# gmh14/tssplat

Measured on AMD Instinct MI355X. Metric: tetrahedra/sec (energy fwd+bwd), higher is better.
Workload: dtype f32

## Files before the change

include/tssplat_amd.h:

```cpp
#ifndef TSSPLAT_AMD_H
#define TSSPLAT_AMD_H

#include <stdint.h>

#ifdef __cplusplus
extern "C" {
#endif

typedef struct tsamd_handle tsamd_handle;

typedef enum tsamd_status {
    TSAMD_OK = 0,
    TSAMD_ERR_INVALID_ARGUMENT = 1,
    TSAMD_ERR_BAD_MESH = 2,
    TSAMD_ERR_NO_DEVICE = 3,
    TSAMD_ERR_HIP = 4,
    TSAMD_ERR_IO = 5,
    TSAMD_ERR_TILING = 6,
    TSAMD_ERR_HOST_ONLY = 7
} tsamd_status;

typedef struct tsamd_options {
    int32_t struct_size;
    int32_t device;
// ... 49 lines not shown
    const float *rest;
} tsamd_tile_view;

const char *tsamd_last_error(void);
const char *tsamd_version(void);
#define TSAMD_ABI_VERSION 3
int32_t tsamd_abi_version(void);

int tsamd_create(const float *rest_xyz, int64_t n_vertices, const int32_t *tets, int64_t n_tets,
                 const tsamd_options *options, tsamd_handle **out);
int tsamd_create_from_veg(const char *path, const tsamd_options *options, tsamd_handle **out);
int tsamd_create_with_operator(const float *rest_xyz, int64_t n_vertices, const int32_t *tets, int64_t n_tets,
                               const int64_t *op_rowptr, const int32_t *op_col, const double *op_val,
                               const tsamd_options *options, tsamd_handle **out);
void tsamd_destroy(tsamd_handle *h);

int64_t tsamd_num_vertices(const tsamd_handle *h);
int64_t tsamd_num_tets(const tsamd_handle *h);
int tsamd_get_plan_info(const tsamd_handle *h, tsamd_plan_info *out);
int tsamd_get_partition_info(const tsamd_handle *h, tsamd_partition_info *out);
int tsamd_get_tile(const tsamd_handle *h, int64_t tile, tsamd_tile_view *out);
int tsamd_get_finish_lists(const tsamd_handle *h, int64_t *n_finish, const int32_t **vid,
                           const int32_t **off, const int32_t **idx);
int tsamd_get_adjacency(const tsamd_handle *h, const int32_t **nbr);

int tsamd_forward(tsamd_handle *h, const float *x_dev, float c1, float c2, int order,
                  void *stream, float *energy_dev);
int tsamd_backward(tsamd_handle *h, const float *x_dev, const float *grad_out_dev, float c1, float c2,
                   int order, void *stream, float *grad_dev);
int tsamd_forward_backward(tsamd_handle *h, const float *x_dev, const float *grad_out_dev, float c1,
                           float c2, int order, void *stream, float *energy_dev, float *grad_dev);
int tsamd_evaluate_dev_coef(tsamd_handle *h, const float *x_dev, const float *grad_out_dev, const float *coef_dev,
                            int order, void *stream, float *energy_dev, float *grad_dev);
typedef struct tsamd_graph tsamd_graph;
int tsamd_graph_create(tsamd_handle *h, const float *x_dev, const float *grad_out_dev, int order, float *energy_dev,
                       float *grad_dev, tsamd_graph **out);
int tsamd_graph_launch(tsamd_graph *graph, float c1, float c2, void *stream);
int tsamd_graph_launch_to(tsamd_graph *graph, float c1, float c2, void *stream, float *energy_copy_dev, float *grad_dev);
void tsamd_graph_destroy(tsamd_graph *graph);

typedef struct tsamd_train_loop tsamd_train_loop;
int64_t tsamd_train_loop_workspace_bytes(int32_t n_iters);
int tsamd_train_loop_create(tsamd_handle *h, float *param_dev, float *grad_dev, float *g1_dev, float *g2_dev, float *energy_ring_dev,
                            void *workspace_dev, int32_t n_iters, tsamd_train_loop **out);
int tsamd_train_loop_launch(tsamd_train_loop *loop, const float *c1, const float *c2, const int32_t *order, float lr, float beta1, float beta2,
                            int64_t first_step, const float *grad_limit, void *stream);
// ... 99 lines not shown
```

tssplat_amd/_capi.py:

```python
from __future__ import annotations

import ctypes as C
import os

from . import _build

_lib = None


class TsamdError(RuntimeError):

    def __init__(self, code: int, message: str):
        super().__init__(f"tssplat_amd error {code}: {message}")
        self.code = code


class Options(C.Structure):
    _fields_ = [
        ("struct_size", C.c_int32),
        ("device", C.c_int32),
        ("lds_budget_bytes", C.c_int32),
        ("max_threads", C.c_int32),
        ("target_owned", C.c_int32),
        ("lane_search_sweeps", C.c_int32),
# ... 34 lines not shown
        ("planes", C.POINTER(C.c_uint32)), ("row_start", C.POINTER(C.c_uint16)),
        ("gvid", C.POINTER(C.c_int32)), ("vdst", C.POINTER(C.c_int32)), ("slot_tet", C.POINTER(C.c_int32)), ("rest", C.POINTER(C.c_float)),
    ]


ABI_VERSION = 3

SIGNATURES = {
    "tsamd_last_error": (C.c_char_p, []),
    "tsamd_version": (C.c_char_p, []),
    "tsamd_abi_version": (C.c_int32, []),
    "tsamd_create": (C.c_int, [C.c_void_p, C.c_int64, C.c_void_p, C.c_int64, C.POINTER(Options), C.POINTER(C.c_void_p)]),
    "tsamd_create_with_operator": (C.c_int, [C.c_void_p, C.c_int64, C.c_void_p, C.c_int64, C.c_void_p, C.c_void_p, C.c_void_p,
                                             C.POINTER(Options), C.POINTER(C.c_void_p)]),
    "tsamd_create_from_veg": (C.c_int, [C.c_char_p, C.POINTER(Options), C.POINTER(C.c_void_p)]),
    "tsamd_destroy": (None, [C.c_void_p]),
    "tsamd_num_vertices": (C.c_int64, [C.c_void_p]),
    "tsamd_num_tets": (C.c_int64, [C.c_void_p]),
    "tsamd_get_plan_info": (C.c_int, [C.c_void_p, C.POINTER(PlanInfo)]),
    "tsamd_get_partition_info": (C.c_int, [C.c_void_p, C.POINTER(PartitionInfo)]),
    "tsamd_get_tile": (C.c_int, [C.c_void_p, C.c_int64, C.POINTER(TileView)]),
    "tsamd_get_finish_lists": (C.c_int, [C.c_void_p, C.POINTER(C.c_int64), C.POINTER(C.POINTER(C.c_int32)),
                                         C.POINTER(C.POINTER(C.c_int32)), C.POINTER(C.POINTER(C.c_int32))]),
    "tsamd_get_adjacency": (C.c_int, [C.c_void_p, C.POINTER(C.POINTER(C.c_int32))]),
    "tsamd_forward": (C.c_int, [C.c_void_p, C.c_void_p, C.c_float, C.c_float, C.c_int, C.c_void_p, C.c_void_p]),
    "tsamd_backward": (C.c_int, [C.c_void_p, C.c_void_p, C.c_void_p, C.c_float, C.c_float, C.c_int, C.c_void_p,
                                 C.c_void_p]),
    "tsamd_forward_backward": (C.c_int, [C.c_void_p, C.c_void_p, C.c_void_p, C.c_float, C.c_float, C.c_int,
                                         C.c_void_p, C.c_void_p, C.c_void_p]),
    "tsamd_evaluate_dev_coef": (C.c_int, [C.c_void_p, C.c_void_p, C.c_void_p, C.c_void_p, C.c_int, C.c_void_p, C.c_void_p,
                                          C.c_void_p]),
    "tsamd_graph_create": (C.c_int, [C.c_void_p, C.c_void_p, C.c_void_p, C.c_int, C.c_void_p, C.c_void_p, C.POINTER(C.c_void_p)]),
    "tsamd_graph_launch": (C.c_int, [C.c_void_p, C.c_float, C.c_float, C.c_void_p]),
    "tsamd_graph_launch_to": (C.c_int, [C.c_void_p, C.c_float, C.c_float, C.c_void_p, C.c_void_p, C.c_void_p]),
    "tsamd_graph_destroy": (None, [C.c_void_p]),
    "tsamd_read_energy_terms": (C.c_int, [C.c_void_p, C.c_void_p, C.POINTER(C.c_double)]),
    "tsamd_set_timing": (C.c_int, [C.c_void_p, C.c_int]),
    "tsamd_get_timing": (C.c_int, [C.c_void_p, C.POINTER(C.c_double), C.POINTER(C.c_double), C.POINTER(C.c_int64)]),
    "tsamd_scale": (C.c_int, [C.c_void_p, C.c_void_p, C.c_void_p, C.c_int64, C.c_void_p]),
    "tsamd_adam_uniform_step": (C.c_int, [C.c_void_p, C.c_void_p, C.c_void_p, C.c_void_p, C.c_int64, C.c_float, C.c_float,
                                        C.c_float, C.c_int64, C.c_float, C.c_void_p, C.c_void_p]),
    "tsamd_grad_limit_workspace_bytes": (C.c_int64, []),
    "tsamd_grad_limit": (C.c_int, [C.c_void_p, C.c_int64, C.c_float, C.c_float, C.c_void_p, C.c_void_p]),
    "tsamd_train_loop_workspace_bytes": (C.c_int64, [C.c_int32]),
    "tsamd_train_loop_create": (C.c_int, [C.c_void_p, C.c_void_p, C.c_void_p, C.c_void_p, C.c_void_p, C.c_void_p, C.c_void_p, C.c_int32,
                                          C.POINTER(C.c_void_p)]),
# ... 128 lines not shown
```

tssplat_amd/csrc/capi.cpp:

```cpp
#include "../../include/tssplat_amd.h"

#include <hip/hip_runtime_api.h>

#include <algorithm>
#include <cmath>
#include <cstdio>
#include <cstdlib>
#include <cstring>
#include <new>
#include <string>
#include <thread>
#include <vector>

#include "capi_common.h"
#include "kernels.h"
#include "plan.h"

namespace {

thread_local std::string g_err;

int fail(int code, const std::string &msg)
{
    g_err = msg;
// ... 60 lines not shown
        for (hipEvent_t e : h->events) (void)hipEventDestroy(e);
    }
    delete h;
}

int to_device(tsamd_handle *h, int device)
{
    int count = 0;
    if (hipGetDeviceCount(&count) != hipSuccess || count <= 0)
        return fail(TSAMD_ERR_NO_DEVICE, "no HIP device is visible (this library has no CPU fallback)");
    if (device < 0) TSAMD_HIP(hipGetDevice(&device));
    if (device >= count) return fail(TSAMD_ERR_INVALID_ARGUMENT, "device ordinal out of range");
    hipDeviceProp_t prop;
    TSAMD_HIP(hipGetDeviceProperties(&prop, device));
    if (size_t(h->plan.lds_bytes) > prop.sharedMemPerBlock && size_t(h->plan.lds_bytes) > prop.maxSharedMemoryPerMultiProcessor)
        return fail(TSAMD_ERR_NO_DEVICE, std::string("device ") + prop.name + " (" + prop.gcnArchName +
                                             ") offers less LDS per workgroup than the plan needs; built for gfx950");
    DeviceGuard g;
    TSAMD_HIP(g.enter(device));
    h->device = device;
    h->host_only = false;
    const tsamd::Plan &P = h->plan;
    int rc;
    if ((rc = upload(h->d_tiles, P.tiles.data(), P.tiles.size(), h->device_bytes))) return rc;
    if (tsamd::planes_paired(P.spt) && !P.tiles.empty()) {
        tsamd::RawVector<uint32_t> image(P.blob.size());
        const int64_t T = int64_t(P.tiles.size());
        const int nthr = int(std::max<int64_t>(1, std::min<int64_t>({int64_t(std::thread::hardware_concurrency()), 64, T / 64 + 1})));
        std::vector<std::thread> pool;
        for (int w = 0; w < nthr; ++w)
            pool.emplace_back([&, w]() {
                for (int64_t t = T * w / nthr; t < T * (w + 1) / nthr; ++t) {
                    const tsamd::TileDesc &d = P.tiles[size_t(t)];
                    const size_t b0 = size_t(d.blob_off / 4), b1 = t + 1 < T ? size_t(P.tiles[size_t(t) + 1].blob_off / 4) : P.blob.size();
                    const size_t np = size_t(P.n_planes) * size_t(d.s_pad);
                    tsamd::interleave_tile_planes(P.blob.data() + b0, image.data() + b0, P.n_planes, d.s_pad, P.spt);
                    std::memcpy(image.data() + b0 + np, P.blob.data() + b0 + np, (b1 - b0 - np) * 4);
                }
            });
        for (auto &th : pool) th.join();
        const size_t head = size_t(P.tiles[0].blob_off / 4);
        if (head) std::memcpy(image.data(), P.blob.data(), head * 4);
        if ((rc = upload(h->d_blob, reinterpret_cast<const uint8_t *>(image.data()), image.size() * 4, h->device_bytes))) return rc;
    } else if ((rc = upload(h->d_blob, reinterpret_cast<const uint8_t *>(P.blob.data()), P.blob.size() * 4, h->device_bytes))) {
        return rc;
    }
    if ((rc = upload(h->d_gvid, P.gvid.data(), P.gvid.size(), h->device_bytes))) return rc;
// ... 17 lines not shown

int create_common(const float *rest, int64_t n, const int32_t *tets, int64_t m, const tsamd_options *o,
                  tsamd_handle **out, const tsamd::ElementOperatorCSR *op = nullptr)
{
    if (!out) return fail(TSAMD_ERR_INVALID_ARGUMENT, "out is null");
    *out = nullptr;
    tsamd_options opt;
    std::memset(&opt, 0, sizeof(opt));
    opt.device = -1;
    if (o) {
        if (o->struct_size != int32_t(sizeof(tsamd_options)))
            return fail(TSAMD_ERR_INVALID_ARGUMENT, "tsamd_options.struct_size does not match this library");
        if (o->abi_version != TSAMD_ABI_VERSION)
            return fail(TSAMD_ERR_INVALID_ARGUMENT, "tsamd_options.abi_version is " + std::to_string(o->abi_version) + ", this library implements ABI " +
                                                        std::to_string(TSAMD_ABI_VERSION) + " (set it to TSAMD_ABI_VERSION of the header you compile against)");
        opt = *o;
    }
    tsamd::PlanOptions po;
    if (opt.lds_budget_bytes > 0) po.lds_budget = opt.lds_budget_bytes;
    if (opt.max_threads > 0) po.max_threads = opt.max_threads;
    po.target_owned = opt.target_owned;
    po.num_threads = opt.num_threads;
    po.conflict_aware = (opt.debug_flags & 2) ? 0 : 1;
    po.lane_search_sweeps = opt.lane_search_sweeps < 0 ? 0 : (opt.lane_search_sweeps == 0 ? 2 : opt.lane_search_sweeps);
    {
        const int spt = opt.slots_per_thread != 0 ? opt.slots_per_thread : tsamd::kSlotsPerLane;
        if (spt < 2 || spt > 4) return fail(TSAMD_ERR_INVALID_ARGUMENT, "slots_per_thread must be 0, 2, 3 or 4");
        if (!tsamd::lane_layout_supported(spt, opt.max_threads > 0 ? opt.max_threads : tsamd::kTileThreads))
            return fail(TSAMD_ERR_INVALID_ARGUMENT, "max_threads exceeds what the tile kernels are compiled for at " + std::to_string(spt) +
                                                        " slots per thread (2: 768, 3: 1024, 4: 768)");
        if (spt != tsamd::kSlotsPerLane && (op || opt.rebuild_dminv == 1))
            return fail(TSAMD_ERR_INVALID_ARGUMENT, "slots_per_thread 3 and 4 are built for the built-in operator with streamed Dm^-1 only");
        po.slots_per_lane = spt;
    }
    if (opt.rebuild_dminv < 0 || opt.rebuild_dminv > 2) return fail(TSAMD_ERR_INVALID_ARGUMENT, "rebuild_dminv must be 0 (auto), 1 (rebuild) or 2 (stream)");
    po.rebuild_dminv = opt.rebuild_dminv == 1 ? 1 : 0;
    tsamd_handle *h = new (std::nothrow) tsamd_handle();
    if (!h) return fail(TSAMD_ERR_INVALID_ARGUMENT, "out of host memory");
    std::string err;
    int rc = 0;
    try {
        rc = tsamd::build_plan(rest, n, tets, m, po, h->plan, err, op);
    } catch (const std::bad_alloc &) {
        rc = TSAMD_ERR_INVALID_ARGUMENT;
        err = "out of host memory while building the plan";
    }
// ... 50 lines not shown
    if (!x && h->plan.n > 0) return fail(TSAMD_ERR_INVALID_ARGUMENT, "x_dev is null");
    return TSAMD_OK;
}

tsamd::EvalArgs eval_args(tsamd_handle *h, const float *x, const float *grad_out, float c1, float c2, int order, float *energy,
                          float *grad, const float *coef)
{
    tsamd::EvalArgs a;
    a.tiles = h->d_tiles;
    a.blob = h->d_blob;
    a.gvid = h->d_gvid;
    a.vdst = h->d_vdst;
    a.fin_vid = h->d_fin_vid;
    a.fin_off = h->d_fin_off;
    a.n_tiles = int64_t(h->plan.tiles.size());
    a.n_finish = int64_t(h->plan.fin_vid.size());
    a.block_threads = h->plan.block_threads;
    a.lds_bytes = h->plan.lds_bytes;
    a.vert_stride = h->plan.vert_stride;
    a.weighted = h->plan.n_planes == tsamd::kPlanesWeighted || h->plan.n_planes == tsamd::kPlanesWeightedSym;
    a.n_planes = h->plan.n_planes;
    a.rebuild = h->plan.n_planes == tsamd::kPlanesRebuild;
    a.spt = h->plan.spt;
    a.x = x;
    a.grad_out = grad_out;
    a.c1 = c1;
    a.c2 = c2;
    a.coef = coef;
    a.order = order;
    a.grad = grad;
    a.stage = h->d_stage;
    a.partials = h->d_partials;
    a.energy = energy;
    a.terms = h->d_terms;
    return a;
}

int evaluate(tsamd_handle *h, const float *x, const float *grad_out, float c1, float c2, int order, void *stream,
             float *energy, float *grad, const float *coef = nullptr)
{
    int rc = check_eval(h, x);
    if (rc) return rc;
    DeviceGuard g;
    TSAMD_HIP(g.enter(h->device));
    const tsamd::EvalArgs a = eval_args(h, x, grad_out, c1, c2, order, energy, grad, coef);
    if (h->timing) {
// ... 95 lines not shown
    if (!h || !out) return fail(TSAMD_ERR_INVALID_ARGUMENT, "null argument");
    const tsamd::Plan &P = h->plan;
    if (tile < 0 || tile >= int64_t(P.tiles.size())) return fail(TSAMD_ERR_INVALID_ARGUMENT, "tile out of range");
    const tsamd::TileDesc &d = P.tiles[size_t(tile)];
    out->n_slots = d.n_slots;
    out->n_owned = d.n_owned;
    out->s_pad = d.s_pad;
    out->n_verts = d.n_verts;
    out->n_excl = d.n_excl;
    out->stage_off = d.stage_off;
    out->n_rows = d.n_rows;
    out->rec_base = d.rec_base;
    out->planes = P.blob.data() + d.blob_off / 4;
    out->row_start = reinterpret_cast<const uint16_t *>(reinterpret_cast<const uint8_t *>(out->planes) + tsamd::tile_rowtab_offset(P.n_planes, d.s_pad));
    out->gvid = P.gvid.data() + d.vert_off;
    out->vdst = P.vdst.data() + d.vert_off;
    out->slot_tet = P.slot_tet.data() + P.slot_base[size_t(tile)];
    out->rest = P.n_planes == tsamd::kPlanesRebuild
                    ? reinterpret_cast<const float *>(reinterpret_cast<const uint8_t *>(out->planes) + tsamd::tile_rest_offset(P.n_planes, d.s_pad))
                    : nullptr;
    return TSAMD_OK;
}

int tsamd_get_finish_lists(const tsamd_handle *h, int64_t *n_finish, const int32_t **vid, const int32_t **off,
                           const int32_t **idx)
{
    if (!h || !n_finish || !vid || !off || !idx) return fail(TSAMD_ERR_INVALID_ARGUMENT, "null argument");
    *n_finish = int64_t(h->plan.fin_vid.size());
    *vid = h->plan.fin_vid.data();
    *off = h->plan.fin_off.data();
    *idx = h->plan.fin_idx.data();
    return TSAMD_OK;
}

int tsamd_get_adjacency(const tsamd_handle *h, const int32_t **nbr)
{
    if (!h || !nbr) return fail(TSAMD_ERR_INVALID_ARGUMENT, "null argument");
    *nbr = h->plan.nbr.data();
    return TSAMD_OK;
}

int tsamd_forward(tsamd_handle *h, const float *x_dev, float c1, float c2, int order, void *stream,
                  float *energy_dev)
{
    if (!energy_dev) return fail(TSAMD_ERR_INVALID_ARGUMENT, "energy_dev is null");
    return evaluate(h, x_dev, nullptr, c1, c2, order, stream, energy_dev, nullptr);
// ... 221 lines not shown
```

tssplat_amd/csrc/kernels.h:

```cpp
#pragma once

#include <hip/hip_runtime_api.h>

#include <cstdint>

#include "plan.h"

namespace tsamd {

struct EvalArgs {
    const TileDesc *tiles;
    const uint8_t *blob;
    const int32_t *gvid, *vdst;
    const int32_t *fin_vid, *fin_off;
    int64_t n_tiles, n_finish;
    int32_t block_threads, lds_bytes;
    int32_t vert_stride = 0;
    bool rebuild = false;
    bool weighted = false;
    int32_t n_planes = 13;
    int32_t spt = kSlotsPerLane;
    const float *x;
    const float *grad_out;
    float c1, c2;
    const float *coef = nullptr;
    int order;
    float *grad;
    float *stage;
    double *partials;
    float *energy;
    double *terms;
};

hipError_t launch_eval(const EvalArgs &a, hipStream_t stream, hipEvent_t *ev = nullptr);
struct EvalGraph;
hipError_t eval_graph_create(const EvalArgs &a, EvalGraph **out);
hipError_t eval_graph_launch(EvalGraph *g, float c1, float c2, hipStream_t stream, float *energy_copy = nullptr, float *grad = nullptr);
void eval_graph_destroy(EvalGraph *g);
struct TrainLoopGraph;
struct TrainLoopStep {
    float c1, c2;
    int order;
    float bias1, bias2, limit;
};
// ... 12 lines not shown
```

tssplat_amd/csrc/kernels.hip:

```cpp
#include <hip/hip_runtime.h>

#include <vector>

#include "kernels.h"

namespace tsamd {
namespace {

constexpr int kWave = 64;

#define SLOT_FENCE() __builtin_amdgcn_sched_barrier(0)
#define STAGE_PRIORITY(n) __builtin_amdgcn_s_setprio(n)
#define UNDEF(x) asm volatile("" : "=v"(x))
typedef uint32_t v4u __attribute__((ext_vector_type(4)));
typedef uint32_t v2u __attribute__((ext_vector_type(2)));

__device__ __forceinline__ float det3(const float *F)
{
    return -F[2] * F[4] * F[6] + F[1] * F[5] * F[6] + F[2] * F[3] * F[7] - F[0] * F[5] * F[7] - F[1] * F[3] * F[8] +
           F[0] * F[4] * F[8];
}

__device__ __forceinline__ void cof3(const float *F, float *C)
{
// ... 173 lines not shown
    const int32_t *gvid;
    const int32_t *vdst;
    const float *x;
    const float *grad_out;
    float *grad;
    float *stage;
    double *partials;
    float c1, c2;
    float ratio;
    const float *coef;
    int order;
    int n_tiles;
    int tiles_per_xcd;
    int vert_stride;
    int n_planes;
};

constexpr uint32_t kXS = kRowTabBytes;
constexpr uint32_t kZeroEntry = 4u * 66u;

__device__ __forceinline__ uint32_t pos_lo(uint32_t w) { return (w & kVertMask) << 4; }
__device__ __forceinline__ uint32_t pos_hi(uint32_t w) { return ((w >> 16) & kVertMask) << 4; }

template <bool WITH_GRAD, bool WEIGHTED, bool REBUILD, int SPT>
__device__ __forceinline__ void tile_body(const KernelArgs &a, const int tile, int32_t gv0)
{
    extern __shared__ __attribute__((aligned(16))) unsigned char smem[];
    typedef uint32_t VU __attribute__((ext_vector_type(SPT)));
    typedef float VF __attribute__((ext_vector_type(SPT)));
    static_assert(!(REBUILD && WEIGHTED), "rebuild_dminv is built for the built-in operator");
    constexpr int kKeepF = SPT, kKeepH = WEIGHTED ? 0 : SPT;
    const TileDesc td = a.tiles[tile];
    const int tid = threadIdx.x, nthr = blockDim.x;
    typedef const __attribute__((address_space(4))) float *ConstF;
    const float k_c1 = a.coef ? ((ConstF)(uintptr_t)a.coef)[0] : a.c1, k_c2 = a.coef ? ((ConstF)(uintptr_t)a.coef)[1] : a.c2;
    const float grad_out_scale = WITH_GRAD && a.grad_out ? *(ConstF)(uintptr_t)a.grad_out : 1.f;
    const auto g_blob = as_global(a.blob);
    const auto g_gvid = as_global(a.gvid);
    const auto g_vdst = as_global(a.vdst);
    const auto g_x = as_global(a.x);
    const auto g_grad = as_global(a.grad);
    const auto g_stage = as_global(a.stage);
    const auto g_partials = as_global(a.partials);
    const uint32_t VP = uint32_t(td.n_verts + 3) & ~3u;
    const uint32_t RS = kXS + 16u * VP;
    const uint32_t RB = uint32_t(td.rec_base);
    LDS_AS double *red = lds_at<double>(RB - 256u);
    const int nq = td.s_pad / SPT;
    const bool active = tid < nq;
    const GLOBAL_AS uint32_t *pl = reinterpret_cast<const GLOBAL_AS uint32_t *>(g_blob + td.blob_off);
    const int lt = active ? tid : 0;
    typedef VU PlaneU __attribute__((aligned(SPT == 3 ? 4 : 4 * SPT)));
    typedef VF PlaneF __attribute__((aligned(SPT == 3 ? 4 : 4 * SPT)));
    auto plane_u = [&](int q) -> VU { return __builtin_nontemporal_load(reinterpret_cast<const GLOBAL_AS PlaneU *>(pl + q * td.s_pad + SPT * lt)); };
    auto plane_f = [&](int q) -> VF { return __builtin_nontemporal_load(reinterpret_cast<const GLOBAL_AS PlaneF *>(pl + q * td.s_pad + SPT * lt)); };
    constexpr bool kPaired = planes_paired(SPT);
    typedef uint32_t VU2 __attribute__((ext_vector_type(2 * SPT)));
    typedef float VF2 __attribute__((ext_vector_type(2 * SPT)));
    auto pair_u = [&](int q, VU &lo, VU &hi) {
        if (kPaired) {
            const VU2 t = __builtin_nontemporal_load(reinterpret_cast<const GLOBAL_AS VU2 *>(pl + q * td.s_pad + 2 * SPT * lt));
#pragma unroll
            for (int p = 0; p < SPT; ++p) lo[p] = t[p], hi[p] = t[SPT + p];
        } else {
            lo = plane_u(q), hi = plane_u(q + 1);
        }
    };
    auto pair_f = [&](int q, VF &lo, VF &hi) {
        if (kPaired) {
            const VF2 t = __builtin_nontemporal_load(reinterpret_cast<const GLOBAL_AS VF2 *>(pl + q * td.s_pad + 2 * SPT * lt));
#pragma unroll
            for (int p = 0; p < SPT; ++p) lo[p] = t[p], hi[p] = t[SPT + p];
        } else {
            lo = plane_f(q), hi = plane_f(q + 1);
        }
    };
    VU q_lv01, q_lv23, q_nb01, q_nb23;
    pair_u(0, q_lv01, q_lv23);
    VF dm[9];
    const int kBasePlanes = REBUILD ? kPlanesRebuild : (WEIGHTED ? a.n_planes : kPlanes);
    const GLOBAL_AS uint16_t *g_rowtab = reinterpret_cast<const GLOBAL_AS uint16_t *>(pl + size_t(kBasePlanes) * td.s_pad);
    const GLOBAL_AS v4f *g_rest = reinterpret_cast<const GLOBAL_AS v4f *>(g_rowtab + kRowTabEntries);
    v4f rest0 = v4f{0.f, 0.f, 0.f, 0.f};
    if (REBUILD) rest0 = g_rest[tid < td.n_verts ? tid : 0];
    __builtin_amdgcn_sched_barrier(0);
    asm volatile("" : "+v"(gv0));
    float px, py, pz;
    {
        const size_t gv = size_t(gv0) * 3;
        px = g_x[gv], py = g_x[gv + 1], pz = g_x[gv + 2];
    }
    __builtin_amdgcn_sched_barrier(0);
    if (!REBUILD) {
#pragma unroll
        for (int c = 0; c < 8; c += 2) pair_f(4 + c, dm[c], dm[c + 1]);
        dm[8] = plane_f(12);
    }
    __builtin_amdgcn_sched_barrier(0);
    if (tid < td.n_verts) {
        *lds_at<v4f>(kXS + 16u * uint32_t(tid)) = v4f{px, py, pz, 0.f};
        if (REBUILD) *lds_at<v4f>(RS + 16u * uint32_t(tid)) = rest0;
    }
    for (int v = tid + nthr; v < td.n_verts; v += nthr) {
        const size_t gv = size_t(g_gvid[td.vert_off + v]) * 3;
        *lds_at<v4f>(kXS + 16u * uint32_t(v)) = v4f{g_x[gv], g_x[gv + 1], g_x[gv + 2], 0.f};
        if (REBUILD) *lds_at<v4f>(RS + 16u * uint32_t(v)) = g_rest[v];
    }
    __syncthreads();
    pair_u(2, q_nb01, q_nb23);
    VF wd, wk[4];
    if (WEIGHTED) {
        wd = plane_f(13);
        pair_f(14, wk[0], wk[1]);
        pair_f(16, wk[2], wk[3]);
    }
    uint32_t row0 = 0;
    if (WITH_GRAD) row0 = __builtin_nontemporal_load(&g_rowtab[tid < 65 ? tid : 64]);
    __builtin_amdgcn_sched_barrier(0);

    const float ratio = a.coef ? k_c2 / k_c1 : a.ratio;
    const bool factored = k_c1 != 0.f && __builtin_fabsf(ratio) <= 0x1p+40f;
    const float s_pen = factored ? ratio : k_c2, out_scale = factored ? k_c1 : 1.f, q_scale = factored ? 1.f : k_c1;
    uint32_t t_own_reg[SPT];
#pragma unroll
    for (int p = 0; p < SPT; ++p) t_own_reg[p] = RB + own_token_addr(uint32_t(p * nq + tid));
    auto t_own_at = [&](int p) -> uint32_t {
        if (!WEIGHTED) return t_own_reg[p];
        uint32_t t = uint32_t(tid);
        asm volatile("" : "+v"(t));
        return RB + own_token_addr(uint32_t(p * nq) + t);
    };
#define t_own(p) t_own_at(p)
    auto is_owned = [&](int p) { return p * nq + tid < td.n_owned; };

    STAGE_PRIORITY(0);
    float scal[SPT];
#pragma unroll
    for (int p = 0; p < SPT; ++p) scal[p] = 0.f;
    float e_b = 0.f, e_s = 0.f;
    float Fk[kKeepF > 0 ? kKeepF : 1][9];
// ... 214 lines not shown
#pragma unroll
                for (int u = 0; u < 4; ++u) {
                    gx += f[u][0];
                    gy += f[u][1];
                    gz += f[u][2];
                }
            }
            if (v < td.n_verts) {
                const bool excl = row >= 0;
                GLOBAL_AS float *dst = (excl ? g_grad : g_stage) + size_t(excl ? row : ~row) * 3;
                const float sc = excl ? gscale : out_scale;
                dst[0] = gx * sc;
                dst[1] = gy * sc;
                dst[2] = gz * sc;
            }
        };
        if (64 * vb0 < td.n_verts) vertex_sums(vb0, dst_row);
        if (64 * nw < td.n_verts) {
            for (int vb = vb0 + nw; 64 * vb < td.n_verts; vb += nw)
                vertex_sums(vb, 64 * vb + lane < td.n_verts ? g_vdst[td.vert_off + 64 * vb + lane] : 0);
        }
    }
#undef t_own
}

template <bool WITH_GRAD, int BLOCK, int WPE, bool WEIGHTED = false, bool REBUILD = false, int SPT = kSlotsPerLane>
__global__ __launch_bounds__(BLOCK, WPE) void tile_energy_kernel(const KernelArgs a)
{
    const int xcd = blockIdx.x & 7, jb = blockIdx.x >> 3;
    const int tile_end = (xcd + 1) * a.tiles_per_xcd < a.n_tiles ? (xcd + 1) * a.tiles_per_xcd : a.n_tiles;
    const int tile = xcd * a.tiles_per_xcd + jb;
    if (jb >= a.tiles_per_xcd || tile >= tile_end) return;
    const int32_t gv0 = __builtin_nontemporal_load(&as_global(a.gvid)[size_t(tile) * size_t(a.vert_stride) + size_t(int(threadIdx.x) < a.vert_stride ? threadIdx.x : 0)]);
    __builtin_amdgcn_sched_barrier(0);
    tile_body<WITH_GRAD, WEIGHTED, REBUILD, SPT>(a, tile, gv0);
}

struct FinishArgs {
    const int32_t *fin_vid, *fin_off;
    int64_t n_finish;
    const float *stage;
    float *grad;
    const float *grad_out;
    const double *partials;
    int64_t n_tiles;
    float c1, c2;
    const float *coef;
    float *energy;
    double *terms;
    float *energy_copy;
};

template <int T>
__device__ __forceinline__ void energy_reduce(const FinishArgs &a, double *red)
{
    const int tid = threadIdx.x;
    const double2 *part = reinterpret_cast<const double2 *>(a.partials);
    double s = 0.0, b = 0.0;
// ... 198 lines not shown
        v.y -= k * a.y;
        v.z -= k * a.z;
        v.w -= k * a.w;
        reinterpret_cast<float4 *>(p)[i] = v;
    }
    for (int64_t i = 4 * n4 + gid; i < n; i += stride) p[i] -= k * g1[i];
}

constexpr int kReduceGridCap = 512;

int grid_for(int64_t n, int per_block, int cap)
{
    int64_t b = (n + per_block - 1) / per_block;
    return int(b < 1 ? 1 : (b > cap ? cap : b));
}

}

hipError_t launch_eval_kernels(const EvalArgs &e, hipStream_t stream, hipEvent_t *ev);

namespace {

#define TSAMD_FN(...) reinterpret_cast<const void *>(&tile_energy_kernel<__VA_ARGS__>)
const void *tile_kernel_for(int spt, int block_threads, bool grad, bool weighted, bool rebuild)
{
    if (spt == 2 && block_threads <= 768) {
        if (weighted) return grad ? TSAMD_FN(true, 768, 6, true, false, 2) : TSAMD_FN(false, 768, 6, true, false, 2);
        if (rebuild) return grad ? TSAMD_FN(true, 768, 6, false, true, 2) : TSAMD_FN(false, 768, 6, false, true, 2);
        return grad ? TSAMD_FN(true, 768, 6, false, false, 2) : TSAMD_FN(false, 768, 6, false, false, 2);
    }
    if (weighted || rebuild) return nullptr;
    if (spt == 3 && block_threads <= 512) return grad ? TSAMD_FN(true, 512, 4, false, false, 3) : TSAMD_FN(false, 512, 4, false, false, 3);
    if (spt == 4 && block_threads <= 768) return grad ? TSAMD_FN(true, 768, 3, false, false, 4) : TSAMD_FN(false, 768, 3, false, false, 4);
    if (spt == 3 && block_threads <= 1024) return grad ? TSAMD_FN(true, 1024, 4, false, false, 3) : TSAMD_FN(false, 1024, 4, false, false, 3);
    return nullptr;
}
#undef TSAMD_FN

}

bool lane_layout_supported(int spt, int max_threads) { return tile_kernel_for(spt, max_threads, true, false, false) != nullptr; }

hipError_t configure_kernels(int lds_bytes)
{
    static int configured[64] = {};
    int dev = 0;
    if (hipGetDevice(&dev) != hipSuccess || dev < 0 || dev >= 64) dev = 0;
    if (lds_bytes <= configured[dev]) return hipSuccess;
    static const int layouts[][2] = {{2, 768}, {3, 512}, {4, 768}, {3, 1024}};
    for (const auto &lay : layouts)
        for (int variant = 0; variant < 6; ++variant) {
            const void *fn = tile_kernel_for(lay[0], lay[1], (variant & 1) != 0, variant / 2 == 1, variant / 2 == 2);
            if (!fn) continue;
            hipFuncAttributes attr;
            hipError_t e = hipFuncGetAttributes(&attr, fn);
            if (e != hipSuccess) return e;
            if (attr.sharedSizeBytes != 0) return hipErrorInvalidDeviceFunction;
            e = hipFuncSetAttribute(fn, hipFuncAttributeMaxDynamicSharedMemorySize, lds_bytes);
            if (e != hipSuccess) return e;
        }
    configured[dev] = lds_bytes;
    return hipSuccess;
}

hipError_t launch_eval(const EvalArgs &e, hipStream_t stream, hipEvent_t *ev)
{
    if (ev) {
        hipError_t err = hipEventRecord(ev[0], stream);
        if (err != hipSuccess) return err;
    }
    hipError_t rc = launch_eval_kernels(e, stream, ev);
    if (rc == hipSuccess && ev) rc = hipEventRecord(ev[2], stream);
    return rc;
}

// ... 14 lines not shown
    k.ratio = c2 / c1;
}

hipError_t make_recipe(const EvalArgs &e, LaunchRecipe &r)
{
    if (e.n_tiles > 0) {
        KernelArgs &k = r.k;
        k.tiles = e.tiles;
        k.blob = e.blob;
        k.gvid = e.gvid;
        k.vdst = e.vdst;
        k.x = e.x;
        k.grad_out = e.grad_out;
        k.grad = e.grad;
        k.stage = e.stage;
        k.partials = e.partials;
        set_coefficients(k, e.c1, e.c2);
        k.coef = e.coef;
        k.order = e.order;
        k.n_tiles = int(e.n_tiles);
        k.tiles_per_xcd = int((e.n_tiles + 7) / 8);
        k.vert_stride = e.vert_stride;
        k.n_planes = e.n_planes;
        r.tile_fn = tile_kernel_for(e.spt, e.block_threads, e.grad != nullptr, e.weighted, e.rebuild);
        if (!r.tile_fn) return hipErrorInvalidConfiguration;
        r.tile_block = dim3(unsigned(e.block_threads));
        r.tile_grid = dim3(unsigned(8 * k.tiles_per_xcd));
        r.tile_lds = size_t(e.lds_bytes);
    }
    FinishArgs &f = r.f;
    f.fin_vid = e.fin_vid;
    f.fin_off = e.fin_off;
    f.n_finish = e.grad ? e.n_finish : 0;
    f.stage = e.stage;
    f.grad = e.grad;
    f.grad_out = e.grad_out;
    f.partials = e.partials;
    f.n_tiles = e.n_tiles;
    f.c1 = e.c1;
    f.c2 = e.c2;
    f.coef = e.coef;
    f.energy = e.energy;
    f.terms = e.terms;
    f.energy_copy = nullptr;
    if (f.n_finish > 0) {
        r.finish_fn = reinterpret_cast<const void *>(&finish_kernel);
        r.finish_grid = dim3(1u + unsigned(grid_for(f.n_finish, 256, 1 << 20)));
// ... 287 lines not shown
```

tssplat_amd/csrc/plan.cpp:

```cpp
#include "plan.h"

#include "conflict_opt.h"
#include "partition.h"

#include <algorithm>
#include <atomic>
#include <cmath>
#include <cstdio>
#include <cstdlib>
#include <cstring>
#include <fstream>
#include <functional>
#include <limits>
#include <numeric>
#include <sstream>
#include <chrono>
#include <thread>

namespace tsamd {
namespace {

struct StageTimer {
    bool on = std::getenv("TSAMD_PLAN_TIMING") != nullptr;
    std::chrono::steady_clock::time_point t0 = std::chrono::steady_clock::now();
// ... 627 lines not shown
            const int64_t k_rcb = int64_t(leaves.size());
            int64_t rcb_slots = 0;
            for (const auto &l : leaves) {
                int64_t ns, nv;
                measure(M, l.data(), int64_t(l.size()), S, ns, nv);
                rcb_slots += ns;
            }
            const int64_t k_lo = (rcb_slots + s_cap - 1) / s_cap;
            CutStats before, after;
            refined[size_t(g)] = partition_component(M, cell_lim, cen.data(), ids, cnt, leaves, k_lo, std::min(k_rcb, k_lo + 3), s_cap, S, cut[size_t(g)], before, after) ? 1 : 0;
        }
    });
    int64_t n_cut = 0, n_refined = 0, n_models = 0;
    for (size_t g = 0; g < groups.size(); ++g) {
        if (model[g] < 0) continue;
        ++n_cut;
        n_models += model[g] == int64_t(g);
        n_refined += refined[size_t(model[g])];
    }
    parallel_chunks(int64_t(groups.size()), 1, nthreads, [&](int64_t b, int64_t e, int w) {
        Scratch &S = get_scratch(w);
        std::vector<int32_t> part;
        for (int64_t g = b; g < e; ++g) {
            const int64_t r = model[size_t(g)];
            if (r < 0 || !refined[size_t(r)]) continue;
            int64_t cnt, cnt_r;
            const int32_t *ids = comp_ids(g, cnt), *ids_r = comp_ids(r, cnt_r);
            auto &leaves = group_tiles[size_t(g)];
            leaves.clear();
            std::string unused_err;
            Splitter sp{M, lim, cen, S, leaves, unused_err};
            for (const auto &c : cut[size_t(r)]) {
                part.resize(c.size());
                for (size_t i = 0; i < c.size(); ++i) part[i] = c[i] - ids_r[0] + ids[0];
                sp.emit(part.data(), int64_t(part.size()));
            }
        }
    });
    P.n_cut_components = n_cut;
    P.n_bisection_components = n_cut - n_refined;
    P.n_cut_templates = n_models;
    if (timer.on)
        std::fprintf(stderr, "[plan] partition: %lld cut components, %lld refined, %lld keep the bisection (%lld cut themselves)\n", (long long)n_cut,
                     (long long)n_refined, (long long)(n_cut - n_refined), (long long)n_models);
    timer.lap("partition (cells + refinement)");
    std::vector<std::vector<int32_t>> tiles_owned;
    for (auto &gt : group_tiles)
        for (auto &t : gt) tiles_owned.push_back(std::move(t));
    group_tiles.clear();
    const int64_t T = int64_t(tiles_owned.size());

    std::vector<std::vector<int32_t>> tile_halo(static_cast<size_t>(T)), tile_verts(static_cast<size_t>(T)), tile_vdeg(static_cast<size_t>(T));
    std::vector<std::atomic<int32_t>> vcount(static_cast<size_t>(n));
    for (auto &a : vcount) a.store(0, std::memory_order_relaxed);
    parallel_chunks(T, 4, nthreads, [&](int64_t b, int64_t e, int w) {
        Scratch &S = get_scratch(w);
        std::vector<int32_t> uniq, cnt;
        std::vector<std::pair<int32_t, int32_t>> key;
        for (int64_t t = b; t < e; ++t) {
// ... 397 lines not shown
                                const int32_t sl = lane_slot[li];
                                uint32_t chosen[4];
                                for (int step = 0; step < 4; ++step) chosen[step] = cand[li][from[li][step]];
                                p2[sl] = record_token(chosen[0], RB) | (record_token(chosen[1], RB) << 16);
                                p3[sl] = record_token(chosen[2], RB) | (record_token(chosen[3], RB) << 16);
                                if (weighted)
                                    for (int base_plane : {14, 18}) {
                                        if (base_plane + 4 > n_planes) continue;
                                        uint32_t old[4];
                                        for (int k = 0; k < 4; ++k) old[k] = pl[size_t(base_plane + k) * size_t(d.s_pad) + sl];
                                        for (int k = 0; k < 4; ++k)
                                            pl[size_t(base_plane + k) * size_t(d.s_pad) + sl] = old[from[li][k]];
                                    }
                            }
                        }
            }
        }
    });
    timer.lap("pass B (planes, ranks, colouring)");
    if (singular.load()) {
        err = "singular (zero-volume) rest tetrahedron";
        return ERR_BAD_MESH;
    }
    return OK;
}

int read_veg(const char *path, std::vector<float> &rest, std::vector<int32_t> &tets, std::string &err)
{
    std::ifstream in(path);
    if (!in) {
        err = std::string("cannot open ") + (path ? path : "(null)");
        return ERR_IO;
    }
    rest.clear();
    tets.clear();
    std::vector<int64_t> ids;
    std::string line;
    int mode = 0, header = 0;
    int64_t min_id = std::numeric_limits<int64_t>::max();
    while (std::getline(in, line)) {
        size_t p = line.find_first_not_of(" \t\r\n");
        if (p == std::string::npos || line[p] == '#') continue;
        if (line[p] == '*') {
            std::string key = line.substr(p);
            for (auto &ch : key) ch = char(std::toupper(static_cast<unsigned char>(ch)));
            if (key.rfind("*VERTICES", 0) == 0) {
// ... 58 lines not shown
```

tssplat_amd/csrc/plan.h:

```cpp
#pragma once

#include <cstdint>
#include <memory>
#include <string>
#include <utility>
#include <vector>

#ifdef __HIPCC__
#define TSAMD_HOST_DEVICE __host__ __device__
#else
#define TSAMD_HOST_DEVICE
#endif

namespace tsamd {

struct PlanOptions {
    int lds_budget = 0;
    int max_threads = 0;
    int target_owned = 0;
    int num_threads = 0;
    int conflict_aware = 1;
    int lane_search_sweeps = 2;
    int rebuild_dminv = 0;
    int slots_per_lane = 0;
};

struct TileDesc {
    uint64_t blob_off;
    int32_t n_slots;
    int32_t n_owned;
    int32_t s_pad;
    int32_t n_verts;
    int32_t n_excl;
    int32_t vert_off;
    int64_t stage_off;
    int32_t n_rows;
    int32_t rec_base;
};
static_assert(sizeof(TileDesc) == 48, "TileDesc layout is part of the kernel ABI");

constexpr int kPlanes = 13;
constexpr int kRowTabEntries = 72;
constexpr int kMaxRank = 64;
constexpr int kSlotsPerLane = 2;
constexpr int kTileThreads = 768;
constexpr int kPlanesWeighted = 22;
constexpr int kPlanesWeightedSym = 18;
// ... 52 lines not shown
            ::new (static_cast<void *>(p)) U(std::forward<Args>(args)...);
    }
};
template <class T>
using RawVector = std::vector<T, DefaultInitAllocator<T>>;

struct Plan {
    int64_t n = 0, m = 0;
    int64_t n_components = 0;
    std::vector<int32_t> nbr;
    std::vector<TileDesc> tiles;
    RawVector<uint32_t> blob;
    RawVector<int32_t> gvid;
    RawVector<int32_t> vdst;
    RawVector<int32_t> slot_tet;
    std::vector<int64_t> slot_base;
    std::vector<int32_t> fin_vid, fin_off, fin_idx;
    int64_t n_stage = 0;
    int64_t total_slots = 0, total_tile_verts = 0;
    int64_t n_cut_components = 0, n_bisection_components = 0, n_cut_templates = 0;
    int32_t max_slots = 0, max_verts = 0, block_threads = 64, lds_bytes = 0, spt = kSlotsPerLane;
    int32_t n_planes = kPlanes;
    int32_t vert_stride = 64;
    std::vector<float> op_diag;
    std::vector<float> op_w;
};

struct ElementOperatorCSR {
    const int64_t *rowptr;
    const int32_t *col;
    const double *val;
};

int build_plan(const float *rest, int64_t n, const int32_t *tets, int64_t m, const PlanOptions &opt,
               Plan &plan, std::string &err, const ElementOperatorCSR *op = nullptr);

int build_adjacency(const int32_t *tets, int64_t n, int64_t m, std::vector<int32_t> &nbr, int nthreads,
                    std::string &err);

int read_veg(const char *path, std::vector<float> &rest, std::vector<int32_t> &tets, std::string &err);

}
```

tssplat_amd/tet_spheres_ext.py:

```python
from __future__ import annotations

import contextlib
import ctypes as C
import os
import sys

import numpy as np
import torch

from . import _capi

__all__ = ["TetSpheres", "forward", "backward", "random_x", "grad_limit"]

_lib = _capi.load()
CPU_ENERGY = os.environ.get("TSSPLAT_AMD_CPU_ENERGY", "0") == "1"
REBUILD_DMINV = {"1": 1, "2": 2}.get(os.environ.get("TSSPLAT_AMD_REBUILD_DMINV", "0"), 0)
print("initializing")


_raw_stream = getattr(torch._C, "_cuda_getCurrentRawStream", None)


def _stream_ptr(device: torch.device) -> int:
    if _raw_stream is not None and device.index is not None:
# ... 82 lines not shown

    def __del__(self):
        try:
            self.close()
        except Exception:
            pass

    def _handle(self):
        if not self._h.value:
            raise RuntimeError("TetSpheres object is empty (construction failed or it was closed)")
        return self._h

    def plan_info(self) -> dict:
        info = _capi.PlanInfo()
        _capi.check(_lib.tsamd_get_plan_info(self._handle(), C.byref(info)))
        out = info.as_dict()
        cut = _capi.PartitionInfo()
        _capi.check(_lib.tsamd_get_partition_info(self._handle(), C.byref(cut)))
        for k, _ in cut._fields_:
            if k != "n_tiles":
                out[k] = getattr(cut, k)
        return out

    def set_timing(self, enable: bool) -> None:
        _capi.check(_lib.tsamd_set_timing(self._handle(), int(enable)))

    def get_timing(self) -> tuple[float, float, int]:
        a, b, n = C.c_double(), C.c_double(), C.c_int64()
        _capi.check(_lib.tsamd_get_timing(self._handle(), C.byref(a), C.byref(b), C.byref(n)))
        return a.value, b.value, n.value

    def energy_terms(self) -> tuple[float, float]:
        out = (C.c_double * 2)()
        _capi.check(_lib.tsamd_read_energy_terms(self._handle(), _stream_ptr(self.device), out))
        return float(out[0]), float(out[1])


def _check_input(x: torch.Tensor, ts: TetSpheres) -> torch.Tensor:
    if not isinstance(x, torch.Tensor):
        raise TypeError("input must be a torch.Tensor")
    if not x.is_cuda:
        raise RuntimeError("tssplat_amd: input must live on the GPU; there is no CPU fallback")
    if ts.device is None or x.device != ts.device:
        raise RuntimeError(f"input is on {x.device} but the TetSpheres object lives on {ts.device}")
    if x.dtype != torch.float32:
        raise RuntimeError("input must be float32")
# ... 71 lines not shown
```

Baseline: 59.23 billion.

## Share identical tile index planes across tiles and load them cached

At plan time, tiles whose index planes and row tables are byte-identical are found by hashing and then confirmed with memcmp. Each duplicate tile's device descriptor points its index reads (stage_off) at the representative tile's blob, and the cut-template leaves are copied by shifting element ids rather than re-emitted per group. When more than half the tiles share index data, a new kernel variant uses ordinary cached loads instead of nontemporal ones, so the shared index planes stay in cache across blocks. The cost is extra plan-time hashing, more kernel instantiations, and reliance on tet meshes made of repeated identical components.

```diff
diff --git a/include/tssplat_amd.h b/include/tssplat_amd.h
--- a/include/tssplat_amd.h
+++ b/include/tssplat_amd.h
@@ -95,6 +95,7 @@
 int tsamd_get_tile(const tsamd_handle *h, int64_t tile, tsamd_tile_view *out);
 int tsamd_get_finish_lists(const tsamd_handle *h, int64_t *n_finish, const int32_t **vid,
                            const int32_t **off, const int32_t **idx);
+int tsamd_get_index_reps(const tsamd_handle *h, const int32_t **rep);
 int tsamd_get_adjacency(const tsamd_handle *h, const int32_t **nbr);
 
 int tsamd_forward(tsamd_handle *h, const float *x_dev, float c1, float c2, int order,
diff --git a/tssplat_amd/_capi.py b/tssplat_amd/_capi.py
--- a/tssplat_amd/_capi.py
+++ b/tssplat_amd/_capi.py
@@ -80,6 +80,7 @@
     "tsamd_get_tile": (C.c_int, [C.c_void_p, C.c_int64, C.POINTER(TileView)]),
     "tsamd_get_finish_lists": (C.c_int, [C.c_void_p, C.POINTER(C.c_int64), C.POINTER(C.POINTER(C.c_int32)),
                                          C.POINTER(C.POINTER(C.c_int32)), C.POINTER(C.POINTER(C.c_int32))]),
+    "tsamd_get_index_reps": (C.c_int, [C.c_void_p, C.POINTER(C.POINTER(C.c_int32))]),
     "tsamd_get_adjacency": (C.c_int, [C.c_void_p, C.POINTER(C.POINTER(C.c_int32))]),
     "tsamd_forward": (C.c_int, [C.c_void_p, C.c_void_p, C.c_float, C.c_float, C.c_int, C.c_void_p, C.c_void_p]),
     "tsamd_backward": (C.c_int, [C.c_void_p, C.c_void_p, C.c_void_p, C.c_float, C.c_float, C.c_int, C.c_void_p,
diff --git a/tssplat_amd/csrc/capi.cpp b/tssplat_amd/csrc/capi.cpp
--- a/tssplat_amd/csrc/capi.cpp
+++ b/tssplat_amd/csrc/capi.cpp
@@ -106,7 +106,11 @@
     h->host_only = false;
     const tsamd::Plan &P = h->plan;
     int rc;
-    if ((rc = upload(h->d_tiles, P.tiles.data(), P.tiles.size(), h->device_bytes))) return rc;
+    {
+        std::vector<tsamd::TileDesc> dev_tiles(P.tiles);
+        for (size_t t = 0; t < dev_tiles.size(); ++t) dev_tiles[t].stage_off = int64_t(P.tiles[size_t(P.index_rep[t])].blob_off);
+        if ((rc = upload(h->d_tiles, dev_tiles.data(), dev_tiles.size(), h->device_bytes))) return rc;
+    }
     if (tsamd::planes_paired(P.spt) && !P.tiles.empty()) {
         tsamd::RawVector<uint32_t> image(P.blob.size());
         const int64_t T = int64_t(P.tiles.size());
@@ -170,6 +174,7 @@
     po.target_owned = opt.target_owned;
     po.num_threads = opt.num_threads;
     po.conflict_aware = (opt.debug_flags & 2) ? 0 : 1;
+    po.share_index = (opt.debug_flags & 4) ? 0 : 1;
     po.lane_search_sweeps = opt.lane_search_sweeps < 0 ? 0 : (opt.lane_search_sweeps == 0 ? 2 : opt.lane_search_sweeps);
     {
         const int spt = opt.slots_per_thread != 0 ? opt.slots_per_thread : tsamd::kSlotsPerLane;
@@ -266,6 +271,7 @@
     a.n_planes = h->plan.n_planes;
     a.rebuild = h->plan.n_planes == tsamd::kPlanesRebuild;
     a.spt = h->plan.spt;
+    a.index_nt = 2 * h->plan.n_index_shared < int64_t(h->plan.tiles.size());
     a.x = x;
     a.grad_out = grad_out;
     a.c1 = c1;
@@ -407,6 +413,13 @@
     return TSAMD_OK;
 }
 
+int tsamd_get_index_reps(const tsamd_handle *h, const int32_t **rep)
+{
+    if (!h || !rep) return fail(TSAMD_ERR_INVALID_ARGUMENT, "null argument");
+    *rep = h->plan.index_rep.data();
+    return TSAMD_OK;
+}
+
 int tsamd_get_finish_lists(const tsamd_handle *h, int64_t *n_finish, const int32_t **vid, const int32_t **off,
                            const int32_t **idx)
 {
diff --git a/tssplat_amd/csrc/kernels.h b/tssplat_amd/csrc/kernels.h
--- a/tssplat_amd/csrc/kernels.h
+++ b/tssplat_amd/csrc/kernels.h
@@ -20,6 +20,7 @@
     bool weighted = false;
     int32_t n_planes = 13;
     int32_t spt = kSlotsPerLane;
+    bool index_nt = true;
     const float *x;
     const float *grad_out;
     float c1, c2;
diff --git a/tssplat_amd/csrc/kernels.hip b/tssplat_amd/csrc/kernels.hip
--- a/tssplat_amd/csrc/kernels.hip
+++ b/tssplat_amd/csrc/kernels.hip
@@ -219,7 +219,7 @@
 __device__ __forceinline__ uint32_t pos_lo(uint32_t w) { return (w & kVertMask) << 4; }
 __device__ __forceinline__ uint32_t pos_hi(uint32_t w) { return ((w >> 16) & kVertMask) << 4; }
 
-template <bool WITH_GRAD, bool WEIGHTED, bool REBUILD, int SPT>
+template <bool WITH_GRAD, bool WEIGHTED, bool REBUILD, int SPT, bool INDEX_NT>
 __device__ __forceinline__ void tile_body(const KernelArgs &a, const int tile, int32_t gv0)
 {
     extern __shared__ __attribute__((aligned(16))) unsigned char smem[];
@@ -249,18 +249,20 @@
     const int lt = active ? tid : 0;
     typedef VU PlaneU __attribute__((aligned(SPT == 3 ? 4 : 4 * SPT)));
     typedef VF PlaneF __attribute__((aligned(SPT == 3 ? 4 : 4 * SPT)));
-    auto plane_u = [&](int q) -> VU { return __builtin_nontemporal_load(reinterpret_cast<const GLOBAL_AS PlaneU *>(pl + q * td.s_pad + SPT * lt)); };
     auto plane_f = [&](int q) -> VF { return __builtin_nontemporal_load(reinterpret_cast<const GLOBAL_AS PlaneF *>(pl + q * td.s_pad + SPT * lt)); };
     constexpr bool kPaired = planes_paired(SPT);
     typedef uint32_t VU2 __attribute__((ext_vector_type(2 * SPT)));
     typedef float VF2 __attribute__((ext_vector_type(2 * SPT)));
+    const GLOBAL_AS uint32_t *pli = reinterpret_cast<const GLOBAL_AS uint32_t *>(g_blob + uint64_t(td.stage_off));
+#define INDEX_LOAD(p) (INDEX_NT ? __builtin_nontemporal_load(p) : *(p))
     auto pair_u = [&](int q, VU &lo, VU &hi) {
         if (kPaired) {
-            const VU2 t = __builtin_nontemporal_load(reinterpret_cast<const GLOBAL_AS VU2 *>(pl + q * td.s_pad + 2 * SPT * lt));
+            const VU2 t = INDEX_LOAD(reinterpret_cast<const GLOBAL_AS VU2 *>(pli + q * td.s_pad + 2 * SPT * lt));
 #pragma unroll
             for (int p = 0; p < SPT; ++p) lo[p] = t[p], hi[p] = t[SPT + p];
         } else {
-            lo = plane_u(q), hi = plane_u(q + 1);
+            lo = INDEX_LOAD(reinterpret_cast<const GLOBAL_AS PlaneU *>(pli + q * td.s_pad + SPT * lt));
+            hi = INDEX_LOAD(reinterpret_cast<const GLOBAL_AS PlaneU *>(pli + (q + 1) * td.s_pad + SPT * lt));
         }
     };
     auto pair_f = [&](int q, VF &lo, VF &hi) {
@@ -276,8 +278,8 @@
     pair_u(0, q_lv01, q_lv23);
     VF dm[9];
     const int kBasePlanes = REBUILD ? kPlanesRebuild : (WEIGHTED ? a.n_planes : kPlanes);
-    const GLOBAL_AS uint16_t *g_rowtab = reinterpret_cast<const GLOBAL_AS uint16_t *>(pl + size_t(kBasePlanes) * td.s_pad);
-    const GLOBAL_AS v4f *g_rest = reinterpret_cast<const GLOBAL_AS v4f *>(g_rowtab + kRowTabEntries);
+    const GLOBAL_AS uint16_t *g_rowtab = reinterpret_cast<const GLOBAL_AS uint16_t *>(pli + size_t(kBasePlanes) * td.s_pad);
+    const GLOBAL_AS v4f *g_rest = reinterpret_cast<const GLOBAL_AS v4f *>(reinterpret_cast<const GLOBAL_AS uint16_t *>(pl + size_t(kBasePlanes) * td.s_pad) + kRowTabEntries);
     v4f rest0 = v4f{0.f, 0.f, 0.f, 0.f};
     if (REBUILD) rest0 = g_rest[tid < td.n_verts ? tid : 0];
     __builtin_amdgcn_sched_barrier(0);
@@ -312,7 +314,7 @@
         pair_f(16, wk[2], wk[3]);
     }
     uint32_t row0 = 0;
-    if (WITH_GRAD) row0 = __builtin_nontemporal_load(&g_rowtab[tid < 65 ? tid : 64]);
+    if (WITH_GRAD) row0 = INDEX_LOAD(&g_rowtab[tid < 65 ? tid : 64]);
     __builtin_amdgcn_sched_barrier(0);
 
     const float ratio = a.coef ? k_c2 / k_c1 : a.ratio;
@@ -573,10 +575,11 @@
         }
     }
 #undef t_own
-}
-
-template <bool WITH_GRAD, int BLOCK, int WPE, bool WEIGHTED = false, bool REBUILD = false, int SPT = kSlotsPerLane>
-__global__ __launch_bounds__(BLOCK, WPE) void tile_energy_kernel(const KernelArgs a)
+#undef INDEX_LOAD
+}
+
+template <bool WITH_GRAD, bool WEIGHTED, bool REBUILD, int SPT, bool INDEX_NT>
+__device__ __forceinline__ void tile_entry(const KernelArgs &a)
 {
     const int xcd = blockIdx.x & 7, jb = blockIdx.x >> 3;
     const int tile_end = (xcd + 1) * a.tiles_per_xcd < a.n_tiles ? (xcd + 1) * a.tiles_per_xcd : a.n_tiles;
@@ -584,7 +587,19 @@
     if (jb >= a.tiles_per_xcd || tile >= tile_end) return;
     const int32_t gv0 = __builtin_nontemporal_load(&as_global(a.gvid)[size_t(tile) * size_t(a.vert_stride) + size_t(int(threadIdx.x) < a.vert_stride ? threadIdx.x : 0)]);
     __builtin_amdgcn_sched_barrier(0);
-    tile_body<WITH_GRAD, WEIGHTED, REBUILD, SPT>(a, tile, gv0);
+    tile_body<WITH_GRAD, WEIGHTED, REBUILD, SPT, INDEX_NT>(a, tile, gv0);
+}
+
+template <bool WITH_GRAD, int BLOCK, int WPE, bool WEIGHTED = false, bool REBUILD = false, int SPT = kSlotsPerLane>
+__global__ __launch_bounds__(BLOCK, WPE) void tile_energy_kernel(const KernelArgs a)
+{
+    tile_entry<WITH_GRAD, WEIGHTED, REBUILD, SPT, true>(a);
+}
+
+template <bool WITH_GRAD, int BLOCK, int WPE, bool WEIGHTED = false, bool REBUILD = false>
+__global__ __launch_bounds__(BLOCK, WPE) void tile_shared_index_kernel(const KernelArgs a)
+{
+    tile_entry<WITH_GRAD, WEIGHTED, REBUILD, kSlotsPerLane, false>(a);
 }
 
 struct FinishArgs {
@@ -829,8 +844,14 @@
 namespace {
 
 #define TSAMD_FN(...) reinterpret_cast<const void *>(&tile_energy_kernel<__VA_ARGS__>)
-const void *tile_kernel_for(int spt, int block_threads, bool grad, bool weighted, bool rebuild)
-{
+#define TSAMD_FN_SHARED(...) reinterpret_cast<const void *>(&tile_shared_index_kernel<__VA_ARGS__>)
+const void *tile_kernel_for(int spt, int block_threads, bool grad, bool weighted, bool rebuild, bool index_nt)
+{
+    if (spt == 2 && block_threads <= 768 && !index_nt) {
+        if (weighted) return grad ? TSAMD_FN_SHARED(true, 768, 6, true, false) : TSAMD_FN_SHARED(false, 768, 6, true, false);
+        if (rebuild) return grad ? TSAMD_FN_SHARED(true, 768, 6, false, true) : TSAMD_FN_SHARED(false, 768, 6, false, true);
+        return grad ? TSAMD_FN_SHARED(true, 768, 6, false, false) : TSAMD_FN_SHARED(false, 768, 6, false, false);
+    }
     if (spt == 2 && block_threads <= 768) {
         if (weighted) return grad ? TSAMD_FN(true, 768, 6, true, false, 2) : TSAMD_FN(false, 768, 6, true, false, 2);
         if (rebuild) return grad ? TSAMD_FN(true, 768, 6, false, true, 2) : TSAMD_FN(false, 768, 6, false, true, 2);
@@ -843,10 +864,11 @@
     return nullptr;
 }
 #undef TSAMD_FN
-
-}
-
-bool lane_layout_supported(int spt, int max_threads) { return tile_kernel_for(spt, max_threads, true, false, false) != nullptr; }
+#undef TSAMD_FN_SHARED
+
+}
+
+bool lane_layout_supported(int spt, int max_threads) { return tile_kernel_for(spt, max_threads, true, false, false, true) != nullptr; }
 
 hipError_t configure_kernels(int lds_bytes)
 {
@@ -856,8 +878,10 @@
     if (lds_bytes <= configured[dev]) return hipSuccess;
     static const int layouts[][2] = {{2, 768}, {3, 512}, {4, 768}, {3, 1024}};
     for (const auto &lay : layouts)
-        for (int variant = 0; variant < 6; ++variant) {
-            const void *fn = tile_kernel_for(lay[0], lay[1], (variant & 1) != 0, variant / 2 == 1, variant / 2 == 2);
+        for (int variant = 0; variant < 12; ++variant) {
+            const int op = (variant % 6) / 2;
+            if (variant >= 6 && lay[0] != kSlotsPerLane) continue;
+            const void *fn = tile_kernel_for(lay[0], lay[1], (variant & 1) != 0, op == 1, op == 2, variant < 6);
             if (!fn) continue;
             hipFuncAttributes attr;
             hipError_t e = hipFuncGetAttributes(&attr, fn);
@@ -918,7 +942,7 @@
         k.tiles_per_xcd = int((e.n_tiles + 7) / 8);
         k.vert_stride = e.vert_stride;
         k.n_planes = e.n_planes;
-        r.tile_fn = tile_kernel_for(e.spt, e.block_threads, e.grad != nullptr, e.weighted, e.rebuild);
+        r.tile_fn = tile_kernel_for(e.spt, e.block_threads, e.grad != nullptr, e.weighted, e.rebuild, e.index_nt);
         if (!r.tile_fn) return hipErrorInvalidConfiguration;
         r.tile_block = dim3(unsigned(e.block_threads));
         r.tile_grid = dim3(unsigned(8 * k.tiles_per_xcd));
diff --git a/tssplat_amd/csrc/plan.cpp b/tssplat_amd/csrc/plan.cpp
--- a/tssplat_amd/csrc/plan.cpp
+++ b/tssplat_amd/csrc/plan.cpp
@@ -673,19 +673,28 @@
         Scratch &S = get_scratch(w);
         std::vector<int32_t> part;
         for (int64_t g = b; g < e; ++g) {
-            const int64_t r = model[size_t(g)];
-            if (r < 0 || !refined[size_t(r)]) continue;
-            int64_t cnt, cnt_r;
-            const int32_t *ids = comp_ids(g, cnt), *ids_r = comp_ids(r, cnt_r);
+            if (model[size_t(g)] != g || !refined[size_t(g)]) continue;
             auto &leaves = group_tiles[size_t(g)];
             leaves.clear();
             std::string unused_err;
             Splitter sp{M, lim, cen, S, leaves, unused_err};
-            for (const auto &c : cut[size_t(r)]) {
-                part.resize(c.size());
-                for (size_t i = 0; i < c.size(); ++i) part[i] = c[i] - ids_r[0] + ids[0];
+            for (const auto &c : cut[size_t(g)]) {
+                part.assign(c.begin(), c.end());
                 sp.emit(part.data(), int64_t(part.size()));
             }
+        }
+    });
+    parallel_chunks(int64_t(groups.size()), 1, nthreads, [&](int64_t b, int64_t e, int) {
+        for (int64_t g = b; g < e; ++g) {
+            const int64_t r = model[size_t(g)];
+            if (r < 0 || r == g) continue;
+            int64_t cnt, cnt_r;
+            const int32_t *ids = comp_ids(g, cnt), *ids_r = comp_ids(r, cnt_r);
+            const int32_t shift = ids[0] - ids_r[0];
+            auto &leaves = group_tiles[size_t(g)];
+            leaves = group_tiles[size_t(r)];
+            for (auto &l : leaves)
+                for (int32_t &el : l) el += shift;
         }
     });
     P.n_cut_components = n_cut;
@@ -1129,6 +1138,47 @@
         err = "singular (zero-volume) rest tetrahedron";
         return ERR_BAD_MESH;
     }
+    P.index_rep.resize(size_t(T));
+    for (int64_t t = 0; t < T; ++t) P.index_rep[size_t(t)] = int32_t(t);
+    if (opt.share_index && T > 1) {
+        const size_t rowtab_words = 2 * kRowTabEntries / 4;
+        auto rowtab_of = [&](const TileDesc &d) { return P.blob.data() + (d.blob_off + uint64_t(tile_rowtab_offset(n_planes, d.s_pad))) / 4; };
+        std::vector<std::pair<uint64_t, int32_t>> by_hash(static_cast<size_t>(T));
+        parallel_chunks(T, 16, nthreads, [&](int64_t b, int64_t e, int) {
+            for (int64_t t = b; t < e; ++t) {
+                const TileDesc &d = P.tiles[size_t(t)];
+                uint64_t h = 1469598103934665603ull;
+                auto mix = [&](uint64_t v) { h = (h ^ v) * 1099511628211ull; };
+                mix(uint64_t(d.s_pad));
+                mix(uint64_t(d.n_slots));
+                mix(uint64_t(d.n_owned));
+                mix(uint64_t(d.n_verts));
+                const uint32_t *pl = P.blob.data() + d.blob_off / 4, *rt = rowtab_of(d);
+                for (size_t i = 0; i < size_t(kPlanesRebuild) * size_t(d.s_pad); ++i) mix(pl[i]);
+                for (size_t i = 0; i < rowtab_words; ++i) mix(rt[i]);
+                by_hash[size_t(t)] = {h, int32_t(t)};
+            }
+        });
+        std::sort(by_hash.begin(), by_hash.end());
+        parallel_chunks(T, 16, nthreads, [&](int64_t b, int64_t e, int) {
+            for (int64_t i = b; i < e; ++i) {
+                const uint64_t h = by_hash[size_t(i)].first;
+                const auto first = std::lower_bound(by_hash.begin(), by_hash.end(), std::make_pair(h, int32_t(0)));
+                const int32_t t = by_hash[size_t(i)].second, r = first->second;
+                if (r == t) continue;
+                const TileDesc &d = P.tiles[size_t(t)], &dr = P.tiles[size_t(r)];
+                if (d.s_pad != dr.s_pad || d.n_slots != dr.n_slots || d.n_owned != dr.n_owned || d.n_verts != dr.n_verts || d.n_rows != dr.n_rows ||
+                    d.rec_base != dr.rec_base)
+                    continue;
+                if (std::memcmp(P.blob.data() + d.blob_off / 4, P.blob.data() + dr.blob_off / 4, size_t(kPlanesRebuild) * size_t(d.s_pad) * 4) != 0 ||
+                    std::memcmp(rowtab_of(d), rowtab_of(dr), 2 * kRowTabEntries) != 0)
+                    continue;
+                P.index_rep[size_t(t)] = r;
+            }
+        });
+        for (int64_t t = 0; t < T; ++t) P.n_index_shared += P.index_rep[size_t(t)] != t;
+    }
+    timer.lap("shared index planes");
     return OK;
 }
 
diff --git a/tssplat_amd/csrc/plan.h b/tssplat_amd/csrc/plan.h
--- a/tssplat_amd/csrc/plan.h
+++ b/tssplat_amd/csrc/plan.h
@@ -23,6 +23,7 @@
     int lane_search_sweeps = 2;
     int rebuild_dminv = 0;
     int slots_per_lane = 0;
+    int share_index = 1;
 };
 
 struct TileDesc {
@@ -121,6 +122,8 @@
     int32_t max_slots = 0, max_verts = 0, block_threads = 64, lds_bytes = 0, spt = kSlotsPerLane;
     int32_t n_planes = kPlanes;
     int32_t vert_stride = 64;
+    std::vector<int32_t> index_rep;
+    int64_t n_index_shared = 0;
     std::vector<float> op_diag;
     std::vector<float> op_w;
 };
diff --git a/tssplat_amd/tet_spheres_ext.py b/tssplat_amd/tet_spheres_ext.py
--- a/tssplat_amd/tet_spheres_ext.py
+++ b/tssplat_amd/tet_spheres_ext.py
@@ -128,6 +128,13 @@
                 out[k] = getattr(cut, k)
         return out
 
+    def index_reps(self):
+        import numpy as np
+        n = self.plan_info()["n_tiles"]
+        p = C.POINTER(C.c_int32)()
+        _capi.check(_lib.tsamd_get_index_reps(self._handle(), C.byref(p)))
+        return np.ctypeslib.as_array(p, shape=(n,)).copy() if n else np.zeros(0, np.int32)
+
     def set_timing(self, enable: bool) -> None:
         _capi.check(_lib.tsamd_set_timing(self._handle(), int(enable)))
 
```

Measured after the change: 63.77 billion, median of 6. 1.08x the previous value.
